# akshatvasisht/janus

Hardware: AMD Instinct MI355X
Metric: xRT (audio-s/wall-s) per GPU, 30s clips batch=64; p50 encode+decode latency (higher is better)
Workload: dtype fp16

## Files before the change

janus_amd/csrc/dec_persist.h:

```cpp
#pragma once
#include "common.h"

namespace janus {

struct DecSegArgs {
  int B, MT;
  float* x;
  const _Float16* o; const _Float16* wo; const float* bo;
  const float* ln2g; const float* ln2b;
  const _Float16* wqk; const float* bqk; _Float16* xqk;
  const _Float16* xc;
  const _Float16* wv; const float* bv; _Float16* omid;
  const _Float16* woc; const float* boc;
  const float* ln3g; const float* ln3b;
  const _Float16* w1; const float* b1; _Float16* f;
  const _Float16* w2; const float* b2;
  const float* ln1g; const float* ln1b;
  const _Float16* wqkv; const float* bqkv; _Float16* qkv;
  _Float16* kc; _Float16* vc; int pos, n_ctx; const int32_t* roff;
  unsigned* bar;
  unsigned* err;
  long long* prof;
  const float* fing; const float* finb; _Float16* fin_out;
  const _Float16* enc; int Te;
};

struct DecSegNext {
  const _Float16* wo; const float* bo;
  const float* ln2g; const float* ln2b;
  const _Float16* wqk; const float* bqk;
};

int dec_seg_mtiles(int B);
int dec_seg_grid(int B, int cus, bool two_per_cu = false);
bool dec_seg_supported(int d, int H, int B, int cus);
bool dec_seg_resident(int grid, int cus);
void dec_seg_a_launch(const DecSegArgs& a, int grid, hipStream_t s);
void dec_seg_b_launch(const DecSegArgs& a, int grid, hipStream_t s);
void dec_layer_launch(const DecSegArgs& b, const DecSegNext& nx, int grid, hipStream_t s);
void dec_head_launch(const DecSegArgs& g, int grid, hipStream_t s);
long long* dec_seg_prof_target(int l);

}
```

janus_amd/csrc/dec_persist.hip:

```cpp
#include "mfma.h"
#include "kernels.h"
#include "dec_persist.h"
#include "xattn_body.h"
#include <algorithm>
#include <cstdlib>

namespace janus {

namespace {

constexpr int kD = 512;
constexpr int kNT = 512;
constexpr int kAP = frag_pitch(kD);
constexpr unsigned kSpinLimit = 1u << 22;

typedef unsigned int u32x4v __attribute__((ext_vector_type(4)));
typedef unsigned int u32x2v __attribute__((ext_vector_type(2)));

__device__ __forceinline__ __amdgpu_buffer_rsrc_t rsrc(const void* p, uint32_t bytes) {
  return __builtin_amdgcn_make_buffer_rsrc(const_cast<void*>(p), 0, bytes, 0x00020000);
}
__device__ __forceinline__ u32x4v ld_sc1(__amdgpu_buffer_rsrc_t r, uint32_t off) {
  return __builtin_amdgcn_raw_buffer_load_b128(r, off, 0, 16);
}
__device__ __forceinline__ void st_sc1(u32x4v v, __amdgpu_buffer_rsrc_t r, uint32_t off) {
  __builtin_amdgcn_raw_buffer_store_b128(v, r, off, 0, 16);
}
__device__ __forceinline__ void st_sc1_8(u32x2v v, __amdgpu_buffer_rsrc_t r, uint32_t off) {
  __builtin_amdgcn_raw_buffer_store_b64(v, r, off, 0, 16);
}
__device__ __forceinline__ half8 as_h8(u32x4v v) { return __builtin_bit_cast(half8, v); }
template <class T>
__device__ __forceinline__ T opaque(T v) {
  asm volatile("" : "+s"(v));
  return v;
}
__device__ __forceinline__ float4 as_f4(u32x4v v) { return __builtin_bit_cast(float4, v); }

#ifdef JANUS_PHASE_PROF
#define SEG_STAMP(ST, I) do { if ((ST) && threadIdx.x == 0) (ST)[I] = (long long)wall_clock64(); } while (0)
#define SEG_END(ST) do { __syncthreads(); SEG_STAMP(ST, 15); } while (0)
#else
#define SEG_STAMP(ST, I) do { (void)(ST); } while (0)
#define SEG_END(ST) do { (void)(ST); } while (0)
#endif

__device__ __forceinline__ void grid_barrier(unsigned* bar, unsigned epoch, unsigned* err,
                                             long long* st = nullptr) {
  asm volatile("s_waitcnt vmcnt(0)" ::: "memory");
  __syncthreads();
  SEG_STAMP(st, 2 * epoch - 1);
  if (threadIdx.x == 0) {
// ... 70 lines not shown
__device__ __forceinline__ int quad_m0() { return 4 * (((int)blockIdx.x >> 3) & 3); }
__device__ __forceinline__ uint32_t touch_quad(const _Float16* wt, int K) {
  return l2_touch(wt + (int64_t)16 * quad_col() * K, (uint32_t)16 * K * 2, ((int)blockIdx.x >> 3) & 3, 4);
}

template <int KSW>
struct SplitW {
  half8 w[KSW];
};

template <int KSW>
__device__ __forceinline__ void splitk_prefetch(SplitW<KSW>& W, const _Float16* wt, int K,
                                                int pair, int MT, int lane, int wv, bool quad = false) {
  const int t = 2 * pair + (wv >> 2), kp = wv & 3;
  const int n = quad ? quad_col() : t / MT;
  const _Float16* wr = wt + (int64_t)(16 * n + (lane & 15)) * K + kp * (K / 4) + 8 * (lane >> 4);
#pragma unroll
  for (int s = 0; s < KSW; ++s) W.w[s] = *reinterpret_cast<const half8*>(wr + 32 * s);
  __builtin_amdgcn_sched_barrier(0);
}

enum SegEpi { SE_RESID = 0, SE_F16_SC1 = 1 };

template <int KSW, int EPI, bool GROUP, class Pre>
__device__ __forceinline__ void splitk_pair(const SplitW<KSW>& W, int pair, int MT, int K,
                                            __amdgpu_buffer_rsrc_t ra, int lda,
                                            const float* bias,
                                            __amdgpu_buffer_rsrc_t rx,
                                            __amdgpu_buffer_rsrc_t ro,
                                            float* red, int lane, int wv, bool last, Pre&& pre,
                                            long long* st = nullptr, int si = 0) {
  const int tsub = wv >> 2, kp = wv & 3;
  const int t = 2 * pair + tsub;
  const int m = t % MT, n = t / MT;
  const int lr = lane & 15, kc8 = 8 * (lane >> 4);
  const int acol = (GROUP ? (16 * n / 64) * kD : 0) + kp * (K / 4) + kc8;
  const uint32_t abase = (uint32_t)(((16 * m + lr) * lda + acol) * 2);
  f32x4 acc = zero_f32x4();
  constexpr int H = KSW > 8 ? 8 : KSW;
#pragma unroll
  for (int h0 = 0; h0 < KSW; h0 += H) {
    half8 a[H];
#pragma unroll
    for (int s = 0; s < H; ++s) a[s] = as_h8(ld_sc1(ra, abase + 64 * (h0 + s)));
#pragma unroll
    for (int s = 0; s < H; ++s) acc = mfma16(a[s], W.w[h0 + s], acc);
    __builtin_amdgcn_sched_barrier(0);
  }
  __builtin_amdgcn_sched_barrier(0);
  if (last) pre();
  __builtin_amdgcn_sched_barrier(0);
  float* rp = red + (tsub * 4 + kp) * 16 * 17;
#pragma unroll
  for (int r = 0; r < 4; ++r) rp[(4 * (lane >> 4) + r) * 17 + lr] = acc[r];
  SEG_STAMP(st, si);
  __syncthreads();
  SEG_STAMP(st, si + 1);
  const int tid = threadIdx.x;
  if (tid < 128) {
    const int es = tid >> 6, q = tid & 63;
    const int et = 2 * pair + es;
    const int em = et % MT, en = et / MT;
    const int row = q >> 2, c4 = 4 * (q & 3);
    const float* r0 = red + (es * 4) * 16 * 17 + row * 17 + c4;
    float v[4];
#pragma unroll
    for (int i = 0; i < 4; ++i) {
      float s = r0[i] + r0[16 * 17 + i];
      s += r0[2 * 16 * 17 + i];
      s += r0[3 * 16 * 17 + i];
      v[i] = s + bias[16 * en + c4 + i];
    }
    const uint32_t eoff = (uint32_t)((16 * em + row) * kD + 16 * en + c4);
    if constexpr (EPI == SE_RESID) {
      const float4 xv = as_f4(ld_sc1(rx, eoff * 4));
      const float4 y = make_float4(xv.x + v[0], xv.y + v[1], xv.z + v[2], xv.w + v[3]);
      st_sc1(__builtin_bit_cast(u32x4v, y), rx, eoff * 4);
    } else {
      const half4 h = {(_Float16)v[0], (_Float16)v[1], (_Float16)v[2], (_Float16)v[3]};
      st_sc1_8(__builtin_bit_cast(u32x2v, h), ro, eoff * 2);
    }
  }
  __syncthreads();
}

struct LngW {
  half8 w[16];
};

template <int MB = 1>
__device__ __forceinline__ void lng_tiles(int N, int MT, int& m, int& nt0, int& npg) {
  const int b = blockIdx.x, G = gridDim.x;
  const int j = b >> 3, xcd = b & 7;
  const int MG = MT / MB;
  const int NG = G / MG;
  m = (j % MG) * MB;
  const int g = xcd + 8 * (j / MG);
  npg = (N / 16) / NG;
  nt0 = g * npg;
}

__device__ __forceinline__ void lng_load(half8 (&w)[16], const _Float16* wt, int nt, int lane) {
  const _Float16* wr = wt + (int64_t)(16 * nt + (lane & 15)) * kD + 8 * (lane >> 4);
#pragma unroll
  for (int s = 0; s < 16; ++s) w[s] = *reinterpret_cast<const half8*>(wr + 32 * s);
// ... 44 lines not shown
  for (int j = 0; j < RW; ++j) {
    const int lrow = RW * wv + j;
    float s = 0.f;
#pragma unroll
    for (int k = 0; k < 2; ++k) s += ln_sum4(v[j][k]);
    s = wave_sum_f32(s);
    const float mean = s / kD;
    float q = 0.f;
#pragma unroll
    for (int k = 0; k < 2; ++k) q += ln_sq4(v[j][k], mean);
    q = wave_sum_f32(q);
    const float rstd = rsqrtf(q / kD + 1e-5f);
#pragma unroll
    for (int k = 0; k < 2; ++k)
      *reinterpret_cast<half4*>(sA + lrow * kAP + 4 * (lane + 64 * k)) = ln_norm4(v[j][k], mean, rstd, gg[k], bb[k]);
  }
  if constexpr (WH < 16) {
#pragma unroll
    for (int k = WH; k < 16; ++k) W.w[k] = *reinterpret_cast<const half8*>(wrow + 32 * k);
  }
  __syncthreads();
  SEG_STAMP(st, si);
  const int lr = lane & 15, kc8 = 8 * (lane >> 4);
  float* patch = patch_all + wv * 16 * 17;
  const int ntile = wv < npg ? (npg - wv + 7) / 8 : 0;
  auto tile = [&](int li, bool last) __attribute__((always_inline)) {
    const int nt = nt0 + li;
    const float4 bias4 = *reinterpret_cast<const float4*>(bias + 16 * nt + 4 * (lane & 3));
    f32x4 acc[MB];
#pragma unroll
    for (int u = 0; u < MB; ++u) acc[u] = zero_f32x4();
    half8 a[2][MB];
#pragma unroll
    for (int u = 0; u < MB; ++u) a[0][u] = *reinterpret_cast<const half8*>(sA + (16 * u + lr) * kAP + kc8);
#pragma unroll
    for (int s = 0; s < 16; ++s) {
      if (s + 1 < 16)
#pragma unroll
        for (int u = 0; u < MB; ++u)
          a[(s + 1) & 1][u] = *reinterpret_cast<const half8*>(sA + (16 * u + lr) * kAP + 32 * (s + 1) + kc8);
#pragma unroll
      for (int u = 0; u < MB; ++u) acc[u] = mfma16(a[s & 1][u], W.w[s], acc[u]);
    }
    if (li == wv) SEG_STAMP(st, si + 1);
    __builtin_amdgcn_sched_barrier(0);
    if (!last) lng_load(W.w, wt, nt + 8, lane);
    else pre();
    __builtin_amdgcn_sched_barrier(0);
#pragma unroll
    for (int u = 0; u < MB; ++u) {
#pragma unroll
    for (int r = 0; r < 4; ++r) patch[(4 * (lane >> 4) + r) * 17 + lr] = acc[u][r];
    __builtin_amdgcn_s_waitcnt(0xc07f);
    const int row = lane >> 2, c4 = 4 * (lane & 3);
    const int grow = 16 * (m + u) + row, col = 16 * nt + c4;
    float v[4];
    v[0] = patch[row * 17 + c4 + 0] + bias4.x;
    v[1] = patch[row * 17 + c4 + 1] + bias4.y;
    v[2] = patch[row * 17 + c4 + 2] + bias4.z;
    v[3] = patch[row * 17 + c4 + 3] + bias4.w;
    if (grow < B) {
      if constexpr (EPI == LE_GELU_SC1) {
        const half4 h = {(_Float16)gelu_erf(v[0]), (_Float16)gelu_erf(v[1]), (_Float16)gelu_erf(v[2]),
                         (_Float16)gelu_erf(v[3])};
        st_sc1_8(__builtin_bit_cast(u32x2v, h), rsrc(o.out, (uint32_t)B * o.ldo * 2),
                 (uint32_t)((grow * o.ldo + col) * 2));
      } else {
        const half4 h = {(_Float16)v[0], (_Float16)v[1], (_Float16)v[2], (_Float16)v[3]};
        if constexpr (EPI == LE_QKV) {
          if (col < kD) {
            st_sc1_8(__builtin_bit_cast(u32x2v, h), rsrc(o.out, (uint32_t)B * o.ldo * 2),
                     (uint32_t)((grow * o.ldo + col) * 2));
          } else {
            _Float16* cache = col < 2 * kD ? o.kc : o.vc;
            const int cpos = o.pos + (o.roff ? o.roff[grow] : 0);
            st_sc1_8(__builtin_bit_cast(u32x2v, h), rsrc(cache, (uint32_t)B * o.n_ctx * kD * 2),
                     (uint32_t)(((grow * o.n_ctx + cpos) * kD + (col % kD)) * 2));
          }
        } else {
          st_sc1_8(__builtin_bit_cast(u32x2v, h), rsrc(o.out, (uint32_t)B * o.ldo * 2),
                   (uint32_t)((grow * o.ldo + col) * 2));
        }
      }
    }
    if (li == wv) SEG_STAMP(st, si + 2);
    }
  };
  for (int i = 0; i + 1 < ntile; ++i) tile(wv + 8 * i, false);
  if (ntile > 0) tile(wv + 8 * (ntile - 1), true);
  else pre();
  (void)N;
}

__device__ __forceinline__ void splitk8_pair(const _Float16* wt, int pair, int MT,
                                             __amdgpu_buffer_rsrc_t ra, const float* bias,
                                             __amdgpu_buffer_rsrc_t rx, float* red, int lane, int wv,
                                             long long* st, int si) {
  constexpr int K = 4 * kD, KS = K / 8 / 32;
  const int t0 = 2 * pair;
  const int m0 = t0 % MT, n = t0 / MT;
  const int lr = lane & 15, kc8 = 8 * (lane >> 4);
  const int k0 = wv * (K / 8) + kc8;
  half8 w[KS], a0[KS], a1[KS];
  const _Float16* wr = wt + (int64_t)(16 * n + lr) * K + k0;
#pragma unroll
  for (int s = 0; s < KS; ++s) w[s] = *reinterpret_cast<const half8*>(wr + 32 * s);
  const uint32_t ab0 = (uint32_t)(((16 * m0 + lr) * K + k0) * 2);
  const uint32_t ab1 = ab0 + (uint32_t)(16 * K * 2);
#pragma unroll
  for (int s = 0; s < KS; ++s) a0[s] = as_h8(ld_sc1(ra, ab0 + 64 * s));
#pragma unroll
  for (int s = 0; s < KS; ++s) a1[s] = as_h8(ld_sc1(ra, ab1 + 64 * s));
  __builtin_amdgcn_sched_barrier(0);
  f32x4 acc0 = zero_f32x4(), acc1 = zero_f32x4();
#pragma unroll
  for (int s = 0; s < KS; ++s) {
    acc0 = mfma16(a0[s], w[s], acc0);
    acc1 = mfma16(a1[s], w[s], acc1);
  }
#pragma unroll
  for (int r = 0; r < 4; ++r) {
    red[((0 * 8 + wv) * 16 + 4 * (lane >> 4) + r) * 17 + lr] = acc0[r];
    red[((1 * 8 + wv) * 16 + 4 * (lane >> 4) + r) * 17 + lr] = acc1[r];
  }
  SEG_STAMP(st, si);
  __syncthreads();
  SEG_STAMP(st, si + 1);
  const int tid = threadIdx.x;
  if (tid < 128) {
    const int es = tid >> 6, q = tid & 63;
    const int em = m0 + es;
    const int row = q >> 2, c4 = 4 * (q & 3);
    const float* r0 = red + (es * 8) * 16 * 17 + row * 17 + c4;
    const float4 b4 = *reinterpret_cast<const float4*>(bias + 16 * n + c4);
    float v[4];
#pragma unroll
    for (int i = 0; i < 4; ++i) {
      float sum = r0[i];
#pragma unroll
      for (int k = 1; k < 8; ++k) sum += r0[k * 16 * 17 + i];
      v[i] = sum;
    }
    v[0] += b4.x; v[1] += b4.y; v[2] += b4.z; v[3] += b4.w;
    const uint32_t eoff = (uint32_t)((16 * em + row) * kD + 16 * n + c4);
    const float4 xv = as_f4(ld_sc1(rx, eoff * 4));
    const float4 y = make_float4(xv.x + v[0], xv.y + v[1], xv.z + v[2], xv.w + v[3]);
    st_sc1(__builtin_bit_cast(u32x4v, y), rx, eoff * 4);
  }
}

template <int KSW, int EPI, bool GROUP, class Pre>
__device__ __forceinline__ void splitk_quad(const SplitW<KSW>& W, int K, __amdgpu_buffer_rsrc_t ra, int lda,
                                            const float* bias, __amdgpu_buffer_rsrc_t rx,
                                            __amdgpu_buffer_rsrc_t ro, float* red, int lane, int wv,
                                            Pre&& pre, long long* st, int si) {
  static_assert(KSW <= 8, "quad split-K: A of both m-tiles in registers");
  const int tsub = wv >> 2, kp = wv & 3;
  const int n = quad_col(), mq = quad_m0();
  const int lr = lane & 15, kc8 = 8 * (lane >> 4);
  const int acol = (GROUP ? (16 * n / 64) * kD : 0) + kp * (K / 4) + kc8;
  half8 a[2][KSW];
#pragma unroll
  for (int v = 0; v < 2; ++v) {
    const uint32_t ab = (uint32_t)(((16 * (mq + 2 * v + tsub) + lr) * lda + acol) * 2);
#pragma unroll
    for (int s = 0; s < KSW; ++s) a[v][s] = as_h8(ld_sc1(ra, ab + 64 * s));
  }
  __builtin_amdgcn_sched_barrier(0);
  f32x4 acc[2] = {zero_f32x4(), zero_f32x4()};
#pragma unroll
  for (int s = 0; s < KSW; ++s)
#pragma unroll
    for (int v = 0; v < 2; ++v) acc[v] = mfma16(a[v][s], W.w[s], acc[v]);
  __builtin_amdgcn_sched_barrier(0);
  pre();
  __builtin_amdgcn_sched_barrier(0);
#pragma unroll
  for (int v = 0; v < 2; ++v) {
    float* rp = red + ((2 * v + tsub) * 4 + kp) * 16 * 17;
#pragma unroll
    for (int r = 0; r < 4; ++r) rp[(4 * (lane >> 4) + r) * 17 + lr] = acc[v][r];
  }
  SEG_STAMP(st, si);
  __syncthreads();
  SEG_STAMP(st, si + 1);
  const int tid = threadIdx.x;
  if (tid < 256) {
    const int es = tid >> 6, q = tid & 63;
    const int em = mq + es;
    const int row = q >> 2, c4 = 4 * (q & 3);
    const float* r0 = red + (es * 4) * 16 * 17 + row * 17 + c4;
    float v[4];
#pragma unroll
    for (int i = 0; i < 4; ++i) {
      float s = r0[i] + r0[16 * 17 + i];
      s += r0[2 * 16 * 17 + i];
      s += r0[3 * 16 * 17 + i];
      v[i] = s + bias[16 * n + c4 + i];
    }
    const uint32_t eoff = (uint32_t)((16 * em + row) * kD + 16 * n + c4);
    if constexpr (EPI == SE_RESID) {
      const float4 xv = as_f4(ld_sc1(rx, eoff * 4));
      const float4 y = make_float4(xv.x + v[0], xv.y + v[1], xv.z + v[2], xv.w + v[3]);
      st_sc1(__builtin_bit_cast(u32x4v, y), rx, eoff * 4);
    } else {
      const half4 h = {(_Float16)v[0], (_Float16)v[1], (_Float16)v[2], (_Float16)v[3]};
      st_sc1_8(__builtin_bit_cast(u32x2v, h), ro, eoff * 2);
    }
  }
  __syncthreads();
}

template <bool PREV>
__device__ __forceinline__ void splitk8_quad(const _Float16* wt, __amdgpu_buffer_rsrc_t ra, const float* bias,
                                             __amdgpu_buffer_rsrc_t rx, float* red, int lane, int wv,
                                             long long* st, int si) {
  constexpr int K = 4 * kD, KS = K / 8 / 32;
  const int n = quad_col(), mq = quad_m0();
  const int lr = lane & 15, kc8 = 8 * (lane >> 4);
  const int k0 = wv * (K / 8) + kc8;
  half8 w[KS], a0[KS], a1[KS];
  const _Float16* wr = wt + (int64_t)(16 * n + lr) * K + k0;
#pragma unroll
  for (int s = 0; s < KS; ++s) w[s] = *reinterpret_cast<const half8*>(wr + 32 * s);
  const int tid = threadIdx.x;
#pragma unroll
  for (int v = 0; v < 2; ++v) {
    const int m0 = mq + 2 * v;
    const uint32_t ab0 = (uint32_t)(((16 * m0 + lr) * K + k0) * 2);
    const uint32_t ab1 = ab0 + (uint32_t)(16 * K * 2);
    if (v == 0 || !PREV) {
#pragma unroll
      for (int s = 0; s < KS; ++s) a0[s] = as_h8(ld_sc1(ra, ab0 + 64 * s));
#pragma unroll
      for (int s = 0; s < KS; ++s) a1[s] = as_h8(ld_sc1(ra, ab1 + 64 * s));
    }
    __builtin_amdgcn_sched_barrier(0);
    f32x4 acc0 = zero_f32x4(), acc1 = zero_f32x4();
#pragma unroll
    for (int s = 0; s < KS; ++s) {
      acc0 = mfma16(a0[s], w[s], acc0);
      acc1 = mfma16(a1[s], w[s], acc1);
    }
    __builtin_amdgcn_sched_barrier(0);
    if (v == 0 && PREV) {
      const uint32_t nb0 = ab0 + (uint32_t)(2 * 16 * K * 2), nb1 = nb0 + (uint32_t)(16 * K * 2);
#pragma unroll
      for (int s = 0; s < KS; ++s) a0[s] = as_h8(ld_sc1(ra, nb0 + 64 * s));
#pragma unroll
      for (int s = 0; s < KS; ++s) a1[s] = as_h8(ld_sc1(ra, nb1 + 64 * s));
      __builtin_amdgcn_sched_barrier(0);
    }
    if (v == 1) __syncthreads();
#pragma unroll
    for (int r = 0; r < 4; ++r) {
      red[((0 * 8 + wv) * 16 + 4 * (lane >> 4) + r) * 17 + lr] = acc0[r];
      red[((1 * 8 + wv) * 16 + 4 * (lane >> 4) + r) * 17 + lr] = acc1[r];
    }
    SEG_STAMP(st, si);
    __syncthreads();
    SEG_STAMP(st, si + 1);
    if (tid < 128) {
      const int es = tid >> 6, q = tid & 63;
      const int em = m0 + es;
      const int row = q >> 2, c4 = 4 * (q & 3);
      const float* r0 = red + (es * 8) * 16 * 17 + row * 17 + c4;
      const float4 b4 = *reinterpret_cast<const float4*>(bias + 16 * n + c4);
      float vv[4];
#pragma unroll
      for (int i = 0; i < 4; ++i) {
        float sum = r0[i];
#pragma unroll
        for (int k = 1; k < 8; ++k) sum += r0[k * 16 * 17 + i];
        vv[i] = sum;
      }
      vv[0] += b4.x; vv[1] += b4.y; vv[2] += b4.z; vv[3] += b4.w;
      const uint32_t eoff = (uint32_t)((16 * em + row) * kD + 16 * n + c4);
      const float4 xv = as_f4(ld_sc1(rx, eoff * 4));
      const float4 y = make_float4(xv.x + vv[0], xv.y + vv[1], xv.z + vv[2], xv.w + vv[3]);
      st_sc1(__builtin_bit_cast(u32x4v, y), rx, eoff * 4);
    }
  }
}

template <int KSW, int EPI, bool GROUP, bool BIG, class Pre>
__device__ __forceinline__ void splitk_phase(const SplitW<KSW>& W, const _Float16* wt, int K,
                                             int MT, __amdgpu_buffer_rsrc_t ra, int lda,
                                             const float* bias, __amdgpu_buffer_rsrc_t rx,
                                             __amdgpu_buffer_rsrc_t ro, float* red, int lane, int wv,
                                             Pre&& pre, long long* st = nullptr, int si = 0) {
  if constexpr (BIG) {
    splitk_quad<KSW, EPI, GROUP>(W, K, ra, lda, bias, rx, ro, red, lane, wv, pre, st, si);
  } else {
    const int p0 = blockIdx.x;
    if (p0 >= 16 * MT) { pre(); return; }
    splitk_pair<KSW, EPI, GROUP>(W, p0, MT, K, ra, lda, bias, rx, ro, red, lane, wv, true, pre, st, si);
  }
  (void)wt;
}

}

constexpr int kRedF = 2 * 8 * 16 * 17;
constexpr int kPatchF = 8 * 16 * 17;
constexpr int kSegRows = 32;
constexpr size_t kSegLds = (size_t)kRedF * 4 + (size_t)kSegRows * kAP * 2 + (size_t)kPatchF * 4;

__device__ __forceinline__ long long* seg_stamps(long long* prof, int k) {
#ifdef JANUS_PHASE_PROF
  if (prof) {
    long long* st = prof + ((int64_t)k * 256 + blockIdx.x) * 48;
    if (threadIdx.x == 0) {
      st[0] = (long long)wall_clock64();
      st[16] = (long long)__builtin_amdgcn_s_getreg((4 << 0) | (0 << 6) | (31 << 11));
      st[17] = (long long)__builtin_amdgcn_s_getreg((20 << 0) | (0 << 6) | (31 << 11));
    }
    return st;
  }
#endif
  (void)prof; (void)k;
  return nullptr;
}

template <bool BIG>
__device__ __forceinline__ void seg_a_body(const DecSegArgs& a, float* seg_smem, long long* st,
                                           long long* pst, unsigned e0, uint32_t& touched,
                                           uint32_t& sink) {
  float* red = seg_smem;
  _Float16* sA = reinterpret_cast<_Float16*>(seg_smem + kRedF);
  float* patch = reinterpret_cast<float*>(sA + kSegRows * kAP);
// ... 47 lines not shown
  sink ^= touched;
  touched = BIG ? touch_lng<2>(a.w1, 4 * kD, MT) : touch_lng<1>(a.w1, 4 * kD, MT);
  {
    SplitW<4> w;
    if (first) splitk_prefetch<4>(w, a.woc, kD, blockIdx.x, MT, lane, wv, BIG);
    splitk_phase<4, SE_RESID, false, BIG>(w, a.woc, kD, MT, rom, kD, a.boc, rx, rx, red, lane, wv, [] {}, pst, 21);
  }
  grid_barrier(a.bar, e0 + 2, a.err, st);
  sink ^= touched;
  touched = BIG ? touch_quad(a.w2, 4 * kD) : touch_splitk(a.w2, 4 * kD, MT);
  {
    LngW w;
    LngOut o{a.f, 4 * kD, nullptr, nullptr, 0, 0, nullptr};
    if constexpr (BIG)
      lng_phase<LE_GELU_SC1, 2>(w, a.w1, 4 * kD, MT, B, rx, a.ln3g, a.ln3b, a.b1, o, sA, patch, lane, wv, [] {}, pst, 24);
    else
      lng_phase<LE_GELU_SC1>(w, a.w1, 4 * kD, MT, B, rx, a.ln3g, a.ln3b, a.b1, o, sA, patch, lane, wv, [] {}, pst, 24);
  }
  grid_barrier(a.bar, e0 + 3, a.err, st);
  sink ^= touched;
  touched = !a.wqkv ? 0u : BIG ? touch_lng<2>(a.wqkv, 3 * kD, MT) : touch_lng<1>(a.wqkv, 3 * kD, MT);
  if (MT % 2 == 0) {
    if constexpr (BIG) {
      splitk8_quad<false>(a.w2, rsrc(a.f, (uint32_t)B * 4 * kD * 2), a.b2, rx, red, lane, wv, pst, 27);
    } else if (first) {
      splitk8_pair(a.w2, blockIdx.x, MT, rsrc(a.f, (uint32_t)B * 4 * kD * 2), a.b2, rx, red, lane, wv, pst, 27);
    }
  } else {
    SplitW<16> w;
    if (first) splitk_prefetch<16>(w, a.w2, 4 * kD, blockIdx.x, MT, lane, wv);
    splitk_phase<16, SE_RESID, false, false>(w, a.w2, 4 * kD, MT, rsrc(a.f, (uint32_t)B * 4 * kD * 2), 4 * kD, a.b2,
                                      rx, rx, red, lane, wv, [] {}, pst, 27);
  }
  if (a.wqkv) {
    grid_barrier(a.bar, e0 + 4, a.err, st);
    sink ^= touched;
    touched = 0u;
    LngW w;
    LngOut o{a.qkv, 3 * kD, a.kc, a.vc, a.pos, a.n_ctx, a.roff};
    if constexpr (BIG)
      lng_phase<LE_QKV, 2>(w, a.wqkv, 3 * kD, MT, B, rx, a.ln1g, a.ln1b, a.bqkv, o, sA, patch, lane, wv, [] {}, pst, 30);
    else
      lng_phase<LE_QKV>(w, a.wqkv, 3 * kD, MT, B, rx, a.ln1g, a.ln1b, a.bqkv, o, sA, patch, lane, wv, [] {}, pst, 30);
  } else if (a.fin_out) {
    grid_barrier(a.bar, e0 + 4, a.err, st);
    sink ^= touched;
    touched = 0u;
// ... 185 lines not shown

constexpr int kXattnLds = XGeo<kD, 64>::LDS;
template <bool BIG>
__device__ __forceinline__ void xattn_phase(const DecSegArgs& g, float* lds) {
  if constexpr (!BIG) {
    const int b = blockIdx.x;
    if (b >= g.B) return;
    xattn_body<kD, 64, false, true, false, true>(g.xqk, g.enc, g.Te, 8, (g.Te + 63) / 64 * 64, nullptr, nullptr,
                                                 nullptr, const_cast<_Float16*>(g.xc), 0, 1, b,
                                                 reinterpret_cast<_Float16*>(lds));
  } else {
    for (int b = blockIdx.x; b < g.B; b += gridDim.x) {
      if (b != (int)blockIdx.x) __syncthreads();
      xattn_body<kD, 64, false, true, false, true>(g.xqk, g.enc, g.Te, 8, (g.Te + 63) / 64 * 64, nullptr, nullptr,
                                                   nullptr, const_cast<_Float16*>(g.xc), 0, 1, b,
                                                   reinterpret_cast<_Float16*>(lds));
    }
  }
}

#define SEG_SINK(A, T, S) do { if (((S) ^ (T)) == 0x5eed5eedu) (A).bar[150] = 1u; } while (0)

template <bool BIG>
__global__ __launch_bounds__(kNT, 4) void dec_seg_a_kernel(DecSegArgs a) {
  JANUS_DEC_WAVE_PRIO();
  extern __shared__ __attribute__((aligned(16))) float seg_smem[];
  long long* st = seg_stamps(a.prof, 0);
  uint32_t touched = 0u, sink = 0u;
  seg_a_body<BIG>(a, seg_smem, st, st, 0, touched, sink);
  SEG_SINK(a, touched, sink);
  SEG_END(st);
  grid_exit(a.bar);
}

template <bool BIG>
__global__ __launch_bounds__(kNT, 4) void dec_seg_b_kernel(DecSegArgs a) {
  JANUS_DEC_WAVE_PRIO();
  extern __shared__ __attribute__((aligned(16))) float seg_smem[];
  long long* st = seg_stamps(a.prof, 1);
  uint32_t touched = 0u, sink = 0u;
  seg_b_body<BIG>(a, seg_smem, st, st, 0, touched, sink);
  SEG_SINK(a, touched, sink);
  SEG_END(st);
  grid_exit(a.bar);
}

template <bool BIG>
__global__ __launch_bounds__(kNT, 4) void dec_layer_kernel(DecSegArgs bsg, DecSegNext nx) {
  JANUS_DEC_WAVE_PRIO();
  extern __shared__ __attribute__((aligned(16))) float seg_smem[];
  long long* st = seg_stamps(bsg.prof, 2);
  const int lane = threadIdx.x & 63, wv = wave_id();
  uint32_t touched = 0u, sink = 0u;
  seg_b_body<BIG>(bsg, seg_smem, st, nullptr, 0, touched, sink);
  grid_barrier(bsg.bar, 5, bsg.err, st);
  sink ^= touched;
  touched = BIG ? touch_quad(nx.wo, kD) : touch_splitk(nx.wo, kD, bsg.MT);
  attn_phase<BIG>(bsg, seg_smem, lane, wv);
  grid_barrier(bsg.bar, 6, bsg.err, st);
  DecSegArgs asg = bsg;
  asg.wo = nx.wo; asg.bo = nx.bo; asg.ln2g = nx.ln2g; asg.ln2b = nx.ln2b; asg.wqk = nx.wqk; asg.bqk = nx.bqk;
  seg_a_body<BIG>(asg, seg_smem, st, nullptr, 6, touched, sink);
  if (bsg.enc) {
    grid_barrier(bsg.bar, 8, bsg.err, st);
    xattn_phase<BIG>(asg, seg_smem);
  }
  SEG_SINK(bsg, touched, sink);
  SEG_END(st);
  grid_exit(bsg.bar);
}

template <bool BIG>
__global__ __launch_bounds__(kNT, 4) void dec_head_kernel(DecSegArgs g) {
  JANUS_DEC_WAVE_PRIO();
  extern __shared__ __attribute__((aligned(16))) float seg_smem[];
  long long* st = seg_stamps(g.prof, 0);
  const int lane = threadIdx.x & 63, wv = wave_id();
  uint32_t touched = 0u, sink = 0u;
  {
    _Float16* sA = reinterpret_cast<_Float16*>(seg_smem + kRedF);
    float* patch = reinterpret_cast<float*>(sA + kSegRows * kAP);
    LngW w;
    LngOut o{g.qkv, 3 * kD, g.kc, g.vc, g.pos, g.n_ctx, g.roff};
    const auto rx0 = rsrc(g.x, (uint32_t)g.B * kD * 4);
    if constexpr (BIG)
      lng_phase<LE_QKV, 2>(w, g.wqkv, 3 * kD, g.MT, g.B, rx0, g.ln1g, g.ln1b, g.bqkv, o, sA, patch, lane, wv,
                           [] {}, nullptr, 30);
    else
      lng_phase<LE_QKV>(w, g.wqkv, 3 * kD, g.MT, g.B, rx0, g.ln1g, g.ln1b, g.bqkv, o, sA, patch, lane, wv,
                        [] {}, nullptr, 30);
  }
  grid_barrier(g.bar, 1, g.err, st);
  touched = BIG ? touch_quad(g.wo, kD) : touch_splitk(g.wo, kD, g.MT);
  attn_phase<BIG>(g, seg_smem, lane, wv);
  grid_barrier(g.bar, 2, g.err, st);
  seg_a_body<BIG>(g, seg_smem, st, nullptr, 2, touched, sink);
  if (g.enc) {
    grid_barrier(g.bar, 4, g.err, st);
    xattn_phase<BIG>(g, seg_smem);
  }
  SEG_SINK(g, touched, sink);
  SEG_END(st);
  grid_exit(g.bar);
}

static int seg_per_cu();

int dec_seg_grid(int B, int cus, bool two_per_cu) {
  const int MT = dec_seg_mtiles(B);
  if (MT <= 0) return 0;
  for (int ng : {32, 16})
    if (MT * ng <= cus) return MT * ng;
  if (MT == 16) {
    if (two_per_cu && 16 * MT <= 2 * cus && seg_per_cu() >= 2) return 16 * MT;
    if (8 * MT <= cus) return 8 * MT;
  }
  return 0;
}

int dec_seg_mtiles(int B) {
  if (B <= 0 || B > 256) return 0;
  int mt = 1;
  while (mt * 16 < B) mt *= 2;
  return mt;
}

bool dec_seg_supported(int d, int H, int B, int cus) {
  return d == kD && H == 8 && dec_seg_grid(B, cus) > 0;
}

static void seg_attr(const void* k, size_t lds = kSegLds) {
  JANUS_HIP(hipFuncSetAttribute(k, hipFuncAttributeMaxDynamicSharedMemorySize, (int)lds));
}

bool dec_seg_resident(int grid, int cus) { return (int64_t)seg_per_cu() * cus >= grid; }

static int seg_per_cu() {
  static int per_cu = -1;
  if (per_cu < 0) {
    const size_t lds = std::max(kSegLds, (size_t)kXattnLds);
    int a = 0, b = 0;
    seg_attr((const void*)dec_layer_kernel<false>, lds);
    seg_attr((const void*)dec_layer_kernel<true>, lds);
    JANUS_HIP(hipOccupancyMaxActiveBlocksPerMultiprocessor(&a, dec_layer_kernel<false>, kNT, lds));
    JANUS_HIP(hipOccupancyMaxActiveBlocksPerMultiprocessor(&b, dec_layer_kernel<true>, kNT, lds));
    per_cu = std::min(a, b);
  }
  return per_cu;
}
static size_t layer_lds(const DecSegArgs& a) {
  return a.enc ? std::max(kSegLds, (size_t)kXattnLds) : kSegLds;
}

static bool seg_big(const DecSegArgs& a, int grid) { return grid < 16 * a.MT; }

template <bool BIG>
static void seg_a_go(const DecSegArgs& a, int grid, hipStream_t s) {
  static bool attr = false;
  if (!attr) { seg_attr((const void*)dec_seg_a_kernel<BIG>); attr = true; }
  dec_seg_a_kernel<BIG><<<grid, kNT, kSegLds, s>>>(a);
  JANUS_LAUNCH_CHECK();
}
void dec_seg_a_launch(const DecSegArgs& a, int grid, hipStream_t s) {
  if (seg_big(a, grid)) seg_a_go<true>(a, grid, s);
  else seg_a_go<false>(a, grid, s);
}

template <bool BIG>
static void seg_b_go(const DecSegArgs& a, int grid, hipStream_t s) {
  static bool attr = false;
  if (!attr) { seg_attr((const void*)dec_seg_b_kernel<BIG>); attr = true; }
  dec_seg_b_kernel<BIG><<<grid, kNT, kSegLds, s>>>(a);
  JANUS_LAUNCH_CHECK();
}
void dec_seg_b_launch(const DecSegArgs& a, int grid, hipStream_t s) {
  if (seg_big(a, grid)) seg_b_go<true>(a, grid, s);
  else seg_b_go<false>(a, grid, s);
// ... 60 lines not shown
```

janus_amd/csrc/whisper.cpp:

```cpp
#include <algorithm>
#include <cstdlib>
#include <map>
#include <condition_variable>
#include <memory>
#include <mutex>
#include <thread>
#include <cstring>
#include "devmem.h"
#include "kernels.h"
#include "decoder.h"
#include "dec_persist.h"
#include "../../include/janus.h"

namespace janus {

struct EncLayer {
  DevMem wqkv, bqkv, wo, w1, w2;
  const float *bo, *b1, *b2, *ln1g, *ln1b, *ln2g, *ln2b;
};
struct DecLayer {
  DevMem wqkv, bqkv, wo, wq_c, wk_c, wv_c, wo_c, w1, w2;
  DevMem wqk, bqk;
  const float *bo, *bq_c, *bv_c, *bo_c, *b1, *b2;
  const float *ln1g, *ln1b, *ln2g, *ln2b, *ln3g, *ln3b;
// ... 526 lines not shown
  Z.d_lncnt.ensure(sizeof(int) * 64);
  JANUS_HIP(hipMemsetAsync(Z.d_lncnt.p, 0, sizeof(int) * 64, s));
  const float* fin_g = w->params.get("decoder.layer_norm.weight", d);
  const float* fin_b = w->params.get("decoder.layer_norm.bias", d);
  auto resid = [&](const _Float16* A, int K, const DevMem& W, const float* bias, const float* ng,
                   const float* nb) {
    GemmArgs g = dgargs(A, K, W.as<_Float16>(), K, bias, x, d, B, d, K, x, d);
    if (fused_ln) g.ln_part = lnp;
    if (ln_fuse) { g.ln_g = ng; g.ln_b = nb; g.ln_out = a; g.ln_cnt = Z.d_lncnt.as<int>(); }
    gemm_launch(EPI_RESID_F32, g, s);
  };
  auto resid_ln = [&](const _Float16* A, const DevMem& W, const float* bias, const float* ng,
                      const float* nb) {
    ResidLnArgs p;
    p.A = A; p.lda = d; p.W = W.as<_Float16>(); p.ldw = d; p.bias = bias;
    p.x = x; p.ldx = d; p.g = ng; p.b = nb; p.eps = 1e-5f; p.out = a;
    p.M = B; p.N = d; p.K = d;
    resid_ln_launch(p, s);
  };
  const bool fuse_se = !path(JANUS_DEC_PATH_NO_SEL_EMBED);
  JANUS_CHECK(!stagger || (!fused_ln && !ln_fuse && !rln && xabs),
              "decode: staggered rows run the default decoder kernels only");
  const int seg_grid = opt->persistent && latch == nullptr ? dec_seg_grid(B, cus, path(JANUS_DEC_PATH_SEG_2CU)) : 0;
  const bool persist = seg_grid > 0 && dec_seg_supported(d, H, B, cus) && dec_seg_resident(seg_grid, cus) &&
                       xabs && !shared && !fused_ln && !ln_fuse && !rln && ngroups == 0 && npairs == 0;
  const bool layerk = persist && opt->persistent >= 2 && 2 * ((B + 1) / 2) <= 2 * seg_grid;
  const bool xfuse = layerk && opt->persistent >= 3 && B <= 2 * seg_grid;
  const bool xrev = !path(JANUS_DEC_PATH_XFWD);
  if (persist) {
    Z.d_omid.ensure(sizeof(_Float16) * B * d);
    if (!Z.d_segbar.p) {
      Z.d_segbar.ensure(sizeof(unsigned) * 256);
      JANUS_HIP(hipMemsetAsync(Z.d_segbar.p, 0, sizeof(unsigned) * 256, s));
    }
    if (!Z.d_segerr.p) {
      Z.d_segerr.ensure(256);
      JANUS_HIP(hipMemsetAsync(Z.d_segerr.p, 0, 256, s));
    }
  }
  auto seg_args = [&](int l, int pos) {
    DecLayer& L = w->dec[l];
    DecSegArgs g{};
    g.B = B; g.MT = dec_seg_mtiles(B); g.x = x;
    g.o = o; g.wo = L.wo.as<_Float16>(); g.bo = L.bo; g.ln2g = L.ln2g; g.ln2b = L.ln2b;
    g.wqk = L.wqk.as<_Float16>(); g.bqk = L.bqk.as<float>(); g.xqk = Z.d_xqk.as<_Float16>();
    g.xc = Z.d_xc.as<_Float16>(); g.wv = L.wv_c.as<_Float16>(); g.bv = L.bv_c; g.omid = Z.d_omid.as<_Float16>();
    g.woc = L.wo_c.as<_Float16>(); g.boc = L.bo_c; g.ln3g = L.ln3g; g.ln3b = L.ln3b;
// ... 517 lines not shown
```

Measured before the change: 6105.

## Hoist split-K epilogue loads before MFMA and widen epilogue stores to 16 bytes

Adds a shared SplitEpi helper that issues the bias and residual loads before the split-K MFMA loop, so their latency overlaps compute instead of landing after the barrier. Fp16 epilogue stores become 128-bit writes of 8 columns instead of 64-bit writes of 4, and the lng tile epilogue writes both m-subtiles through a larger LDS patch buffer. splitk8_quad now loads all four A row tiles up front and runs the MFMAs in one pass. The BIG kernels get launch_bounds of 2 waves per EU, giving them more registers, and residency is now checked per variant. The risks are higher register pressure and more LDS, which may lower occupancy.

```diff
diff --git a/janus_amd/csrc/dec_persist.h b/janus_amd/csrc/dec_persist.h
--- a/janus_amd/csrc/dec_persist.h
+++ b/janus_amd/csrc/dec_persist.h
@@ -34,7 +34,7 @@
 int dec_seg_mtiles(int B);
 int dec_seg_grid(int B, int cus, bool two_per_cu = false);
 bool dec_seg_supported(int d, int H, int B, int cus);
-bool dec_seg_resident(int grid, int cus);
+bool dec_seg_resident(int B, int grid, int cus);
 void dec_seg_a_launch(const DecSegArgs& a, int grid, hipStream_t s);
 void dec_seg_b_launch(const DecSegArgs& a, int grid, hipStream_t s);
 void dec_layer_launch(const DecSegArgs& b, const DecSegNext& nx, int grid, hipStream_t s);
diff --git a/janus_amd/csrc/dec_persist.hip b/janus_amd/csrc/dec_persist.hip
--- a/janus_amd/csrc/dec_persist.hip
+++ b/janus_amd/csrc/dec_persist.hip
@@ -15,7 +15,6 @@
 constexpr unsigned kSpinLimit = 1u << 22;
 
 typedef unsigned int u32x4v __attribute__((ext_vector_type(4)));
-typedef unsigned int u32x2v __attribute__((ext_vector_type(2)));
 
 __device__ __forceinline__ __amdgpu_buffer_rsrc_t rsrc(const void* p, uint32_t bytes) {
   return __builtin_amdgcn_make_buffer_rsrc(const_cast<void*>(p), 0, bytes, 0x00020000);
@@ -25,9 +24,6 @@
 }
 __device__ __forceinline__ void st_sc1(u32x4v v, __amdgpu_buffer_rsrc_t r, uint32_t off) {
   __builtin_amdgcn_raw_buffer_store_b128(v, r, off, 0, 16);
-}
-__device__ __forceinline__ void st_sc1_8(u32x2v v, __amdgpu_buffer_rsrc_t r, uint32_t off) {
-  __builtin_amdgcn_raw_buffer_store_b64(v, r, off, 0, 16);
 }
 __device__ __forceinline__ half8 as_h8(u32x4v v) { return __builtin_bit_cast(half8, v); }
 template <class T>
@@ -144,6 +140,52 @@
 
 enum SegEpi { SE_RESID = 0, SE_F16_SC1 = 1 };
 
+template <int EPI>
+struct SplitEpi {
+  static constexpr int CW = EPI == SE_RESID ? 4 : 8;
+  static constexpr int TPT = 256 / CW;
+  int es, row, c0;
+  bool active;
+  float b[CW];
+  u32x4v x;
+
+  __device__ __forceinline__ SplitEpi(int tid, int NT)
+      : es((tid / TPT) & (NT - 1)), row((tid % TPT) / (16 / CW)), c0(CW * (tid % (16 / CW))),
+        active(tid < NT * TPT) {}
+  __device__ __forceinline__ uint32_t eoff(int em, int en) const {
+    return (uint32_t)((16 * em + row) * kD + 16 * en + c0);
+  }
+  __device__ __forceinline__ void issue(int em, int en, const float* bias, __amdgpu_buffer_rsrc_t rx) {
+#pragma unroll
+    for (int i = 0; i < CW; ++i) b[i] = bias[16 * en + c0 + i];
+    if constexpr (EPI == SE_RESID) x = ld_sc1(rx, active ? eoff(em, en) * 4 : 0x80000000u);
+  }
+  template <int NPART>
+  __device__ __forceinline__ void finish(const float* red, int em, int en, __amdgpu_buffer_rsrc_t rx,
+                                         __amdgpu_buffer_rsrc_t ro) const {
+    if (!active) return;
+    const float* r0 = red + (es * NPART) * 16 * 17 + row * 17 + c0;
+    float v[CW];
+#pragma unroll
+    for (int i = 0; i < CW; ++i) {
+      float s = r0[i];
+#pragma unroll
+      for (int k = 1; k < NPART; ++k) s += r0[k * 16 * 17 + i];
+      v[i] = s + b[i];
+    }
+    if constexpr (EPI == SE_RESID) {
+      const float4 xv = as_f4(x);
+      const float4 y = make_float4(xv.x + v[0], xv.y + v[1], xv.z + v[2], xv.w + v[3]);
+      st_sc1(__builtin_bit_cast(u32x4v, y), rx, eoff(em, en) * 4);
+    } else {
+      half8 h;
+#pragma unroll
+      for (int i = 0; i < CW; ++i) h[i] = (_Float16)v[i];
+      st_sc1(__builtin_bit_cast(u32x4v, h), ro, eoff(em, en) * 2);
+    }
+  }
+};
+
 template <int KSW, int EPI, bool GROUP, class Pre>
 __device__ __forceinline__ void splitk_pair(const SplitW<KSW>& W, int pair, int MT, int K,
                                             __amdgpu_buffer_rsrc_t ra, int lda,
@@ -158,6 +200,10 @@
   const int lr = lane & 15, kc8 = 8 * (lane >> 4);
   const int acol = (GROUP ? (16 * n / 64) * kD : 0) + kp * (K / 4) + kc8;
   const uint32_t abase = (uint32_t)(((16 * m + lr) * lda + acol) * 2);
+  SplitEpi<EPI> ep(threadIdx.x, 2);
+  const int et = 2 * pair + ep.es;
+  const int em = et % MT, en = et / MT;
+  if constexpr (KSW <= 8) ep.issue(em, en, bias, rx);
   f32x4 acc = zero_f32x4();
   constexpr int H = KSW > 8 ? 8 : KSW;
 #pragma unroll
@@ -170,6 +216,7 @@
     __builtin_amdgcn_sched_barrier(0);
   }
   __builtin_amdgcn_sched_barrier(0);
+  if constexpr (KSW > 8) ep.issue(em, en, bias, rx);
   if (last) pre();
   __builtin_amdgcn_sched_barrier(0);
   float* rp = red + (tsub * 4 + kp) * 16 * 17;
@@ -178,31 +225,7 @@
   SEG_STAMP(st, si);
   __syncthreads();
   SEG_STAMP(st, si + 1);
-  const int tid = threadIdx.x;
-  if (tid < 128) {
-    const int es = tid >> 6, q = tid & 63;
-    const int et = 2 * pair + es;
-    const int em = et % MT, en = et / MT;
-    const int row = q >> 2, c4 = 4 * (q & 3);
-    const float* r0 = red + (es * 4) * 16 * 17 + row * 17 + c4;
-    float v[4];
-#pragma unroll
-    for (int i = 0; i < 4; ++i) {
-      float s = r0[i] + r0[16 * 17 + i];
-      s += r0[2 * 16 * 17 + i];
-      s += r0[3 * 16 * 17 + i];
-      v[i] = s + bias[16 * en + c4 + i];
-    }
-    const uint32_t eoff = (uint32_t)((16 * em + row) * kD + 16 * en + c4);
-    if constexpr (EPI == SE_RESID) {
-      const float4 xv = as_f4(ld_sc1(rx, eoff * 4));
-      const float4 y = make_float4(xv.x + v[0], xv.y + v[1], xv.z + v[2], xv.w + v[3]);
-      st_sc1(__builtin_bit_cast(u32x4v, y), rx, eoff * 4);
-    } else {
-      const half4 h = {(_Float16)v[0], (_Float16)v[1], (_Float16)v[2], (_Float16)v[3]};
-      st_sc1_8(__builtin_bit_cast(u32x2v, h), ro, eoff * 2);
-    }
-  }
+  ep.template finish<4>(red, em, en, rx, ro);
   __syncthreads();
 }
 
@@ -293,11 +316,13 @@
   __syncthreads();
   SEG_STAMP(st, si);
   const int lr = lane & 15, kc8 = 8 * (lane >> 4);
-  float* patch = patch_all + wv * 16 * 17;
+  float* patch = patch_all + wv * 2 * 16 * 17;
+  const int c8 = 8 * (lane & 1);
   const int ntile = wv < npg ? (npg - wv + 7) / 8 : 0;
   auto tile = [&](int li, bool last) __attribute__((always_inline)) {
     const int nt = nt0 + li;
-    const float4 bias4 = *reinterpret_cast<const float4*>(bias + 16 * nt + 4 * (lane & 3));
+    const float4 bias8[2] = {*reinterpret_cast<const float4*>(bias + 16 * nt + c8),
+                             *reinterpret_cast<const float4*>(bias + 16 * nt + c8 + 4)};
     f32x4 acc[MB];
 #pragma unroll
     for (int u = 0; u < MB; ++u) acc[u] = zero_f32x4();
@@ -319,43 +344,32 @@
     else pre();
     __builtin_amdgcn_sched_barrier(0);
 #pragma unroll
-    for (int u = 0; u < MB; ++u) {
-#pragma unroll
-    for (int r = 0; r < 4; ++r) patch[(4 * (lane >> 4) + r) * 17 + lr] = acc[u][r];
+    for (int u = 0; u < MB; ++u)
+#pragma unroll
+      for (int r = 0; r < 4; ++r) patch[(16 * u + 4 * (lane >> 4) + r) * 17 + lr] = acc[u][r];
     __builtin_amdgcn_s_waitcnt(0xc07f);
-    const int row = lane >> 2, c4 = 4 * (lane & 3);
-    const int grow = 16 * (m + u) + row, col = 16 * nt + c4;
-    float v[4];
-    v[0] = patch[row * 17 + c4 + 0] + bias4.x;
-    v[1] = patch[row * 17 + c4 + 1] + bias4.y;
-    v[2] = patch[row * 17 + c4 + 2] + bias4.z;
-    v[3] = patch[row * 17 + c4 + 3] + bias4.w;
-    if (grow < B) {
-      if constexpr (EPI == LE_GELU_SC1) {
-        const half4 h = {(_Float16)gelu_erf(v[0]), (_Float16)gelu_erf(v[1]), (_Float16)gelu_erf(v[2]),
-                         (_Float16)gelu_erf(v[3])};
-        st_sc1_8(__builtin_bit_cast(u32x2v, h), rsrc(o.out, (uint32_t)B * o.ldo * 2),
-                 (uint32_t)((grow * o.ldo + col) * 2));
+    const int eu = MB == 2 ? lane >> 5 : 0;
+    const int row = (lane & 31) >> 1;
+    const int grow = 16 * (m + eu) + row, col = 16 * nt + c8;
+    const float* pr = patch + (16 * eu + row) * 17 + c8;
+    float v[8];
+    v[0] = pr[0] + bias8[0].x; v[1] = pr[1] + bias8[0].y; v[2] = pr[2] + bias8[0].z; v[3] = pr[3] + bias8[0].w;
+    v[4] = pr[4] + bias8[1].x; v[5] = pr[5] + bias8[1].y; v[6] = pr[6] + bias8[1].z; v[7] = pr[7] + bias8[1].w;
+    if (grow < B && (MB == 2 || lane < 32)) {
+      half8 h;
+#pragma unroll
+      for (int i = 0; i < 8; ++i) h[i] = (_Float16)(EPI == LE_GELU_SC1 ? gelu_erf(v[i]) : v[i]);
+      const u32x4v hv = __builtin_bit_cast(u32x4v, h);
+      if (EPI == LE_QKV && col >= kD) {
+        _Float16* cache = col < 2 * kD ? o.kc : o.vc;
+        const int cpos = o.pos + (o.roff ? o.roff[grow] : 0);
+        st_sc1(hv, rsrc(cache, (uint32_t)B * o.n_ctx * kD * 2),
+               (uint32_t)(((grow * o.n_ctx + cpos) * kD + (col % kD)) * 2));
       } else {
-        const half4 h = {(_Float16)v[0], (_Float16)v[1], (_Float16)v[2], (_Float16)v[3]};
-        if constexpr (EPI == LE_QKV) {
-          if (col < kD) {
-            st_sc1_8(__builtin_bit_cast(u32x2v, h), rsrc(o.out, (uint32_t)B * o.ldo * 2),
-                     (uint32_t)((grow * o.ldo + col) * 2));
-          } else {
-            _Float16* cache = col < 2 * kD ? o.kc : o.vc;
-            const int cpos = o.pos + (o.roff ? o.roff[grow] : 0);
-            st_sc1_8(__builtin_bit_cast(u32x2v, h), rsrc(cache, (uint32_t)B * o.n_ctx * kD * 2),
-                     (uint32_t)(((grow * o.n_ctx + cpos) * kD + (col % kD)) * 2));
-          }
-        } else {
-          st_sc1_8(__builtin_bit_cast(u32x2v, h), rsrc(o.out, (uint32_t)B * o.ldo * 2),
-                   (uint32_t)((grow * o.ldo + col) * 2));
-        }
+        st_sc1(hv, rsrc(o.out, (uint32_t)B * o.ldo * 2), (uint32_t)((grow * o.ldo + col) * 2));
       }
     }
     if (li == wv) SEG_STAMP(st, si + 2);
-    }
   };
   for (int i = 0; i + 1 < ntile; ++i) tile(wv + 8 * i, false);
   if (ntile > 0) tile(wv + 8 * (ntile - 1), true);
@@ -389,6 +403,10 @@
     acc0 = mfma16(a0[s], w[s], acc0);
     acc1 = mfma16(a1[s], w[s], acc1);
   }
+  __builtin_amdgcn_sched_barrier(0);
+  SplitEpi<SE_RESID> ep(threadIdx.x, 2);
+  ep.issue(m0 + ep.es, n, bias, rx);
+  __builtin_amdgcn_sched_barrier(0);
 #pragma unroll
   for (int r = 0; r < 4; ++r) {
     red[((0 * 8 + wv) * 16 + 4 * (lane >> 4) + r) * 17 + lr] = acc0[r];
@@ -397,27 +415,7 @@
   SEG_STAMP(st, si);
   __syncthreads();
   SEG_STAMP(st, si + 1);
-  const int tid = threadIdx.x;
-  if (tid < 128) {
-    const int es = tid >> 6, q = tid & 63;
-    const int em = m0 + es;
-    const int row = q >> 2, c4 = 4 * (q & 3);
-    const float* r0 = red + (es * 8) * 16 * 17 + row * 17 + c4;
-    const float4 b4 = *reinterpret_cast<const float4*>(bias + 16 * n + c4);
-    float v[4];
-#pragma unroll
-    for (int i = 0; i < 4; ++i) {
-      float sum = r0[i];
-#pragma unroll
-      for (int k = 1; k < 8; ++k) sum += r0[k * 16 * 17 + i];
-      v[i] = sum;
-    }
-    v[0] += b4.x; v[1] += b4.y; v[2] += b4.z; v[3] += b4.w;
-    const uint32_t eoff = (uint32_t)((16 * em + row) * kD + 16 * n + c4);
-    const float4 xv = as_f4(ld_sc1(rx, eoff * 4));
-    const float4 y = make_float4(xv.x + v[0], xv.y + v[1], xv.z + v[2], xv.w + v[3]);
-    st_sc1(__builtin_bit_cast(u32x4v, y), rx, eoff * 4);
-  }
+  ep.template finish<8>(red, m0 + ep.es, n, rx, rx);
 }
 
 template <int KSW, int EPI, bool GROUP, class Pre>
@@ -437,6 +435,8 @@
 #pragma unroll
     for (int s = 0; s < KSW; ++s) a[v][s] = as_h8(ld_sc1(ra, ab + 64 * s));
   }
+  SplitEpi<EPI> ep(threadIdx.x, 4);
+  ep.issue(mq + ep.es, n, bias, rx);
   __builtin_amdgcn_sched_barrier(0);
   f32x4 acc[2] = {zero_f32x4(), zero_f32x4()};
 #pragma unroll
@@ -455,34 +455,10 @@
   SEG_STAMP(st, si);
   __syncthreads();
   SEG_STAMP(st, si + 1);
-  const int tid = threadIdx.x;
-  if (tid < 256) {
-    const int es = tid >> 6, q = tid & 63;
-    const int em = mq + es;
-    const int row = q >> 2, c4 = 4 * (q & 3);
-    const float* r0 = red + (es * 4) * 16 * 17 + row * 17 + c4;
-    float v[4];
-#pragma unroll
-    for (int i = 0; i < 4; ++i) {
-      float s = r0[i] + r0[16 * 17 + i];
-      s += r0[2 * 16 * 17 + i];
-      s += r0[3 * 16 * 17 + i];
-      v[i] = s + bias[16 * n + c4 + i];
-    }
-    const uint32_t eoff = (uint32_t)((16 * em + row) * kD + 16 * n + c4);
-    if constexpr (EPI == SE_RESID) {
-      const float4 xv = as_f4(ld_sc1(rx, eoff * 4));
-      const float4 y = make_float4(xv.x + v[0], xv.y + v[1], xv.z + v[2], xv.w + v[3]);
-      st_sc1(__builtin_bit_cast(u32x4v, y), rx, eoff * 4);
-    } else {
-      const half4 h = {(_Float16)v[0], (_Float16)v[1], (_Float16)v[2], (_Float16)v[3]};
-      st_sc1_8(__builtin_bit_cast(u32x2v, h), ro, eoff * 2);
-    }
-  }
+  ep.template finish<4>(red, mq + ep.es, n, rx, ro);
   __syncthreads();
 }
 
-template <bool PREV>
 __device__ __forceinline__ void splitk8_quad(const _Float16* wt, __amdgpu_buffer_rsrc_t ra, const float* bias,
                                              __amdgpu_buffer_rsrc_t rx, float* red, int lane, int wv,
                                              long long* st, int si) {
@@ -490,67 +466,38 @@
   const int n = quad_col(), mq = quad_m0();
   const int lr = lane & 15, kc8 = 8 * (lane >> 4);
   const int k0 = wv * (K / 8) + kc8;
-  half8 w[KS], a0[KS], a1[KS];
+  half8 w[KS], a[4][KS];
   const _Float16* wr = wt + (int64_t)(16 * n + lr) * K + k0;
 #pragma unroll
   for (int s = 0; s < KS; ++s) w[s] = *reinterpret_cast<const half8*>(wr + 32 * s);
-  const int tid = threadIdx.x;
+#pragma unroll
+  for (int u = 0; u < 4; ++u) {
+    const uint32_t ab = (uint32_t)(((16 * (mq + u) + lr) * K + k0) * 2);
+#pragma unroll
+    for (int s = 0; s < KS; ++s) a[u][s] = as_h8(ld_sc1(ra, ab + 64 * s));
+  }
+  SplitEpi<SE_RESID> ep[2] = {SplitEpi<SE_RESID>(threadIdx.x, 2), SplitEpi<SE_RESID>(threadIdx.x, 2)};
+#pragma unroll
+  for (int v = 0; v < 2; ++v) ep[v].issue(mq + 2 * v + ep[v].es, n, bias, rx);
+  __builtin_amdgcn_sched_barrier(0);
+  f32x4 acc[4] = {zero_f32x4(), zero_f32x4(), zero_f32x4(), zero_f32x4()};
+#pragma unroll
+  for (int s = 0; s < KS; ++s)
+#pragma unroll
+    for (int u = 0; u < 4; ++u) acc[u] = mfma16(a[u][s], w[s], acc[u]);
+  __builtin_amdgcn_sched_barrier(0);
 #pragma unroll
   for (int v = 0; v < 2; ++v) {
-    const int m0 = mq + 2 * v;
-    const uint32_t ab0 = (uint32_t)(((16 * m0 + lr) * K + k0) * 2);
-    const uint32_t ab1 = ab0 + (uint32_t)(16 * K * 2);
-    if (v == 0 || !PREV) {
-#pragma unroll
-      for (int s = 0; s < KS; ++s) a0[s] = as_h8(ld_sc1(ra, ab0 + 64 * s));
-#pragma unroll
-      for (int s = 0; s < KS; ++s) a1[s] = as_h8(ld_sc1(ra, ab1 + 64 * s));
-    }
-    __builtin_amdgcn_sched_barrier(0);
-    f32x4 acc0 = zero_f32x4(), acc1 = zero_f32x4();
-#pragma unroll
-    for (int s = 0; s < KS; ++s) {
-      acc0 = mfma16(a0[s], w[s], acc0);
-      acc1 = mfma16(a1[s], w[s], acc1);
-    }
-    __builtin_amdgcn_sched_barrier(0);
-    if (v == 0 && PREV) {
-      const uint32_t nb0 = ab0 + (uint32_t)(2 * 16 * K * 2), nb1 = nb0 + (uint32_t)(16 * K * 2);
-#pragma unroll
-      for (int s = 0; s < KS; ++s) a0[s] = as_h8(ld_sc1(ra, nb0 + 64 * s));
-#pragma unroll
-      for (int s = 0; s < KS; ++s) a1[s] = as_h8(ld_sc1(ra, nb1 + 64 * s));
-      __builtin_amdgcn_sched_barrier(0);
-    }
     if (v == 1) __syncthreads();
 #pragma unroll
     for (int r = 0; r < 4; ++r) {
-      red[((0 * 8 + wv) * 16 + 4 * (lane >> 4) + r) * 17 + lr] = acc0[r];
-      red[((1 * 8 + wv) * 16 + 4 * (lane >> 4) + r) * 17 + lr] = acc1[r];
+      red[((0 * 8 + wv) * 16 + 4 * (lane >> 4) + r) * 17 + lr] = acc[2 * v][r];
+      red[((1 * 8 + wv) * 16 + 4 * (lane >> 4) + r) * 17 + lr] = acc[2 * v + 1][r];
     }
     SEG_STAMP(st, si);
     __syncthreads();
     SEG_STAMP(st, si + 1);
-    if (tid < 128) {
-      const int es = tid >> 6, q = tid & 63;
-      const int em = m0 + es;
-      const int row = q >> 2, c4 = 4 * (q & 3);
-      const float* r0 = red + (es * 8) * 16 * 17 + row * 17 + c4;
-      const float4 b4 = *reinterpret_cast<const float4*>(bias + 16 * n + c4);
-      float vv[4];
-#pragma unroll
-      for (int i = 0; i < 4; ++i) {
-        float sum = r0[i];
-#pragma unroll
-        for (int k = 1; k < 8; ++k) sum += r0[k * 16 * 17 + i];
-        vv[i] = sum;
-      }
-      vv[0] += b4.x; vv[1] += b4.y; vv[2] += b4.z; vv[3] += b4.w;
-      const uint32_t eoff = (uint32_t)((16 * em + row) * kD + 16 * n + c4);
-      const float4 xv = as_f4(ld_sc1(rx, eoff * 4));
-      const float4 y = make_float4(xv.x + vv[0], xv.y + vv[1], xv.z + vv[2], xv.w + vv[3]);
-      st_sc1(__builtin_bit_cast(u32x4v, y), rx, eoff * 4);
-    }
+    ep[v].template finish<8>(red, mq + 2 * v + ep[v].es, n, rx, rx);
   }
 }
 
@@ -573,10 +520,11 @@
 }
 
 constexpr int kRedF = 2 * 8 * 16 * 17;
-constexpr int kPatchF = 8 * 16 * 17;
+constexpr int kPatchF = 8 * 2 * 16 * 17;
 constexpr int kSegRows = 32;
 constexpr size_t kSegLds = (size_t)kRedF * 4 + (size_t)kSegRows * kAP * 2 + (size_t)kPatchF * 4;
 
+constexpr int seg_waves(bool big) { return big ? 2 : 4; }
 __device__ __forceinline__ long long* seg_stamps(long long* prof, int k) {
 #ifdef JANUS_PHASE_PROF
   if (prof) {
@@ -670,7 +618,7 @@
   touched = !a.wqkv ? 0u : BIG ? touch_lng<2>(a.wqkv, 3 * kD, MT) : touch_lng<1>(a.wqkv, 3 * kD, MT);
   if (MT % 2 == 0) {
     if constexpr (BIG) {
-      splitk8_quad<false>(a.w2, rsrc(a.f, (uint32_t)B * 4 * kD * 2), a.b2, rx, red, lane, wv, pst, 27);
+      splitk8_quad(a.w2, rsrc(a.f, (uint32_t)B * 4 * kD * 2), a.b2, rx, red, lane, wv, pst, 27);
     } else if (first) {
       splitk8_pair(a.w2, blockIdx.x, MT, rsrc(a.f, (uint32_t)B * 4 * kD * 2), a.b2, rx, red, lane, wv, pst, 27);
     }
@@ -902,7 +850,7 @@
 #define SEG_SINK(A, T, S) do { if (((S) ^ (T)) == 0x5eed5eedu) (A).bar[150] = 1u; } while (0)
 
 template <bool BIG>
-__global__ __launch_bounds__(kNT, 4) void dec_seg_a_kernel(DecSegArgs a) {
+__global__ __launch_bounds__(kNT, seg_waves(BIG)) void dec_seg_a_kernel(DecSegArgs a) {
   JANUS_DEC_WAVE_PRIO();
   extern __shared__ __attribute__((aligned(16))) float seg_smem[];
   long long* st = seg_stamps(a.prof, 0);
@@ -914,7 +862,7 @@
 }
 
 template <bool BIG>
-__global__ __launch_bounds__(kNT, 4) void dec_seg_b_kernel(DecSegArgs a) {
+__global__ __launch_bounds__(kNT, seg_waves(BIG)) void dec_seg_b_kernel(DecSegArgs a) {
   JANUS_DEC_WAVE_PRIO();
   extern __shared__ __attribute__((aligned(16))) float seg_smem[];
   long long* st = seg_stamps(a.prof, 1);
@@ -926,7 +874,7 @@
 }
 
 template <bool BIG>
-__global__ __launch_bounds__(kNT, 4) void dec_layer_kernel(DecSegArgs bsg, DecSegNext nx) {
+__global__ __launch_bounds__(kNT, seg_waves(BIG)) void dec_layer_kernel(DecSegArgs bsg, DecSegNext nx) {
   JANUS_DEC_WAVE_PRIO();
   extern __shared__ __attribute__((aligned(16))) float seg_smem[];
   long long* st = seg_stamps(bsg.prof, 2);
@@ -951,7 +899,7 @@
 }
 
 template <bool BIG>
-__global__ __launch_bounds__(kNT, 4) void dec_head_kernel(DecSegArgs g) {
+__global__ __launch_bounds__(kNT, seg_waves(BIG)) void dec_head_kernel(DecSegArgs g) {
   JANUS_DEC_WAVE_PRIO();
   extern __shared__ __attribute__((aligned(16))) float seg_smem[];
   long long* st = seg_stamps(g.prof, 0);
@@ -984,7 +932,7 @@
   grid_exit(g.bar);
 }
 
-static int seg_per_cu();
+static int seg_per_cu(bool big);
 
 int dec_seg_grid(int B, int cus, bool two_per_cu) {
   const int MT = dec_seg_mtiles(B);
@@ -992,7 +940,7 @@
   for (int ng : {32, 16})
     if (MT * ng <= cus) return MT * ng;
   if (MT == 16) {
-    if (two_per_cu && 16 * MT <= 2 * cus && seg_per_cu() >= 2) return 16 * MT;
+    if (two_per_cu && 16 * MT <= 2 * cus && seg_per_cu(false) >= 2) return 16 * MT;
     if (8 * MT <= cus) return 8 * MT;
   }
   return 0;
@@ -1013,26 +961,28 @@
   JANUS_HIP(hipFuncSetAttribute(k, hipFuncAttributeMaxDynamicSharedMemorySize, (int)lds));
 }
 
-bool dec_seg_resident(int grid, int cus) { return (int64_t)seg_per_cu() * cus >= grid; }
-
-static int seg_per_cu() {
+static bool seg_big(int MT, int grid) { return grid < 16 * MT; }
+
+bool dec_seg_resident(int B, int grid, int cus) {
+  return (int64_t)seg_per_cu(seg_big(dec_seg_mtiles(B), grid)) * cus >= grid;
+}
+
+template <bool BIG>
+static int seg_per_cu_of() {
   static int per_cu = -1;
   if (per_cu < 0) {
     const size_t lds = std::max(kSegLds, (size_t)kXattnLds);
-    int a = 0, b = 0;
-    seg_attr((const void*)dec_layer_kernel<false>, lds);
-    seg_attr((const void*)dec_layer_kernel<true>, lds);
-    JANUS_HIP(hipOccupancyMaxActiveBlocksPerMultiprocessor(&a, dec_layer_kernel<false>, kNT, lds));
-    JANUS_HIP(hipOccupancyMaxActiveBlocksPerMultiprocessor(&b, dec_layer_kernel<true>, kNT, lds));
-    per_cu = std::min(a, b);
+    seg_attr((const void*)dec_layer_kernel<BIG>, lds);
+    JANUS_HIP(hipOccupancyMaxActiveBlocksPerMultiprocessor(&per_cu, dec_layer_kernel<BIG>, kNT, lds));
   }
   return per_cu;
 }
+static int seg_per_cu(bool big) { return big ? seg_per_cu_of<true>() : seg_per_cu_of<false>(); }
 static size_t layer_lds(const DecSegArgs& a) {
   return a.enc ? std::max(kSegLds, (size_t)kXattnLds) : kSegLds;
 }
 
-static bool seg_big(const DecSegArgs& a, int grid) { return grid < 16 * a.MT; }
+static bool seg_big(const DecSegArgs& a, int grid) { return seg_big(a.MT, grid); }
 
 template <bool BIG>
 static void seg_a_go(const DecSegArgs& a, int grid, hipStream_t s) {
diff --git a/janus_amd/csrc/whisper.cpp b/janus_amd/csrc/whisper.cpp
--- a/janus_amd/csrc/whisper.cpp
+++ b/janus_amd/csrc/whisper.cpp
@@ -572,7 +572,7 @@
   JANUS_CHECK(!stagger || (!fused_ln && !ln_fuse && !rln && xabs),
               "decode: staggered rows run the default decoder kernels only");
   const int seg_grid = opt->persistent && latch == nullptr ? dec_seg_grid(B, cus, path(JANUS_DEC_PATH_SEG_2CU)) : 0;
-  const bool persist = seg_grid > 0 && dec_seg_supported(d, H, B, cus) && dec_seg_resident(seg_grid, cus) &&
+  const bool persist = seg_grid > 0 && dec_seg_supported(d, H, B, cus) && dec_seg_resident(B, seg_grid, cus) &&
                        xabs && !shared && !fused_ln && !ln_fuse && !rln && ngroups == 0 && npairs == 0;
   const bool layerk = persist && opt->persistent >= 2 && 2 * ((B + 1) / 2) <= 2 * seg_grid;
   const bool xfuse = layerk && opt->persistent >= 3 && B <= 2 * seg_grid;
```

Measured after the change: 6137 (median of 6 runs). About the same (+0.5%).
